# SpaceLearner/SessionRec-pytorch

Hardware: AMD Instinct MI355X
Metric: sessions/sec training, Yoochoose-1/64 batch 512 (higher is better)
Workload: dtype bf16 (MFMA operands; fp32 accumulate, master weights, scoring); 1 GPU; MSGIFSR training step, synthetic Yoochoose-1/64 shape (V=37484 items, d=256, batch 512 per GPU, session length<=20, order 3, dropout 0.1); global_batch=512, parallelism=single GPU

## Files before the change

### include/srec.h

```cpp
#ifndef SREC_H
#define SREC_H
#include "srec_hg.h"

#ifdef __cplusplus
extern "C" {
#endif

#define SREC_BAD_ARG 1001

int srec_gemm_f32(const float* A, int a_rs, int a_cs, const float* B, int b_rs, int b_cs, float* C, int ldc,
                  const float* bias, int M, int N, int K, const int* dyn, int dyn_mode, float alpha, float beta,
                  float* ws, long ws_floats, void* stream);

int srec_gemm_bf16_nt(const float* A, int lda, const float* B, int ldb, float* C, int ldc, const float* bias, int M,
                      int N, int K, const int* dyn, float alpha, float beta, float* ws, long ws_floats, void* stream);

int srec_gemm_bf16_tn(const float* A, int lda, const float* B, int ldb, float* C, int ldc, int Mred, int N, int K,
                      const int* dyn, float alpha, float beta, float* ws, long ws_floats, void* stream);

int srec_ce_plan(int B, int V, int d, int* n_item_tiles, int* n_ranges);
int srec_score_ce_fwd(const float* sr, int ld_sr, const float* E, int ld_e, const float* cs, const int* labels,
                      int B, int V, int d, const int* dynB, float* ws_stats, float* lab_logit, float* lse,
                      float* lossvec, float* loss, void* stream);
int srec_score_ce_bwd(const float* sr, int ld_sr, const float* E, int ld_e, const float* cs, const int* labels,
// ... 152 lines not shown
int srec_adam_hyper_multi(int n, const void* counter, const void* cfg, const void* hyper, const int* tap_counter,
                          const float* tap_src, float* tap_ring, int tap_n, const int* skip, void* stream);
typedef struct srec_adam_multi_desc {
    int nt;
    const int* use_wd;
    const long* numel;
    float* const* p;
    const float* const* g;
    float* const* m;
    float* const* v;
} srec_adam_multi_desc;
int srec_adam_multi(const void* desc, const float* hyper, void* stream);
int srec_adam_rows(float* W, const float* G, float* M, float* V, int n, int d, int ld, const float* hyper,
                   int use_wd, float max_norm, int renorm_write, float* cs_out, float cs_scale, int eps_mode,
                   float cs_eps, void* dst16, int Dp, void* stream);
int srec_adam_rows_proj(float* W, const float* G, float* M, float* V, int n, int d, int ld, const float* hyper, int use_wd,
                        float max_norm, int renorm_write, float* cs_out, float cs_scale, int eps_mode, float cs_eps,
                        const float* proj_cs, float proj_inv_scale, float* radial, void* dst16, int Dp, void* stream);
int srec_adam_rows_lookup(float* W, const float* G, float* M, float* V, int n, int d, int ld, const float* hyper, int use_wd,
                          float max_norm, int renorm_write, float* cs_out, float cs_scale, int eps_mode, float cs_eps,
                          const float* proj_cs, float proj_inv_scale, float* radial, void* dst16, int Dp, int* slot,
                          const float* part, const int* cptr, int u_cap, int n_part, void* stream);
int srec_adam_rows_multi(float* W, const float* G, float* M, float* V, int n, int d, int ld, const float* hyper, int use_wd,
                         float max_norm, int renorm_write, float* cs_out, float cs_scale, int eps_mode, float cs_eps,
                         const float* proj_cs, float proj_inv_scale, float* radial, void* dst16, int Dp, int* slot,
                         const float* part, const int* cptr, int u_cap, int n_part, const void* desc, const float* multi_hyper,
                         void* stream);

int srec_hg_ws_floats(const void* desc, long* n_floats);
int srec_hg_fwd(const void* desc, const float* x, int ld_x, float* out, int ld_out, unsigned char* arg, void* stream);
int srec_hg_fold(const void* desc, void* stream);
int srec_step_prep(const void* desc, void* stream);
int srec_hg_drop_prep(const float* x, const float* cnt, int rows, int D, float p, int seed, const int* counter, int salt,
                      float* ms, float* xc, float* rm, float* xres, float pa, long na, float* mk, void* stream);
int srec_hg_drop_prep16(const float* x, const float* cnt, int rows, int D, float p, int seed, const int* counter, int salt,
                        float* ms, float* xc, float* rm, float* xres, float pa, long na, float* mk, void* xc16, void* stream);
int srec_hg_live_rows(const void* desc, const void* lists, int* counts, void* stream);
int srec_hg_drop_prep16_live(const float* x, const float* cnt, int rows, int D, float p, int seed, const int* counter, int salt,
                             float* ms, float* xc, float* rm, float* xres, float pa, long na, float* mk, void* xc16,
                             const void* desc, const void* lists, int* counts, void* stream);
int srec_hg_drop_merge(const float* t, int S, const float* ms, long n, float* dx, float p, int seed, const int* counter,
                       int salt, void* stream);
int srec_hg_pre_merge(const void* desc, const float* g, int ld_g, const float* t, int S, float* dx, int ld_dx, void* stream);
int srec_hg_bwd(const void* desc, const float* x, int ld_x, const float* g, int ld_g, const unsigned char* arg, float* dx,
                int ld_dx, float* ws, void* stream);

int srec_gemm_group_bf16(const void* desc, int mode, void* stream);

int srec_gemm_f32_group_run(const void* desc, float* ws, long ws_floats, void* stream);
int srec_gemm_f32_group_run_defer(const void* desc, float* ws, long ws_floats, long* slab_off, int* slab_n, void* stream);
int srec_gemm16_nt(const void* desc, void* stream);
int srec_gemm16_nt_rows(const void* desc, const void* rows, void* stream);
int srec_gemm16_tn(const void* desc, void* stream);
int srec_rows_bf16(const float* src, int ld, int n, const int* dyn, int d, void* dst16, void* stream);
int srec_sum_slabs(const float* part, int C, int R, long n, float* out, void* stream);
int srec_weights_bf16(int n, const void* W, const void* W16, const void* WT16, const int* R, const int* Cc, void* stream);
int srec_norm_perm_pick_fwd(const float* x, int ld_x, const int* perm, int n_cap, const int* dyn_t, int D, int eps_mode,
                            float eps, float* allf, float* invr, int npick, int B, const int* dyn_b, const void* pick,
                            const void* pout, const int* ld_p, void* stream);
int srec_norm_perm_pick_bwd(const float* allf, const float* invr, const float* g_allf, int ld_g, const int* perm, int n_cap,
                            const int* cat_seg, int B, const int* dyn_b, int D, int npick, const void* pick, const void* g_pick,
                            const int* ld_gp, float* dx, int ld_dx, int nt, const int* row0, const int* ncap, const void* dyn_n,
                            int n_rows, void* stream);
int srec_gru_step_fwd(const void* desc, void* stream);
int srec_gru_step_bwd(const void* desc, void* stream);
int srec_gru_fused_fwd(const void* desc, void* stream);
int srec_gru_wfrag(int n, const void* W, const void* dst, int d, void* stream);
int srec_gru_fused_bwd(const void* desc, void* stream);
int srec_gru_fused_nodes(int np, const int* n, int d, int* nodes);
int srec_gru_fused_wide(int np, const int* n, const int* k, int* mask);
int srec_gru_fused_waves(int d, int* waves);
int srec_gru_wfrag_t(int n, const void* W, const void* dst, int d, void* stream);
int srec_gru_wfrag_both(int n, const void* W, const void* dst_fwd, const void* dst_bwd, int d, void* stream);
int srec_gru_bias_final(int np, const void* part, const int* rows, int ncol, const void* out, void* stream);
int srec_sum_slabs_multi(int np, const void* part, const int* R, const long* n, const void* out, const int* tall,
                         void* stream);
int srec_sum_slabs_multi_ld(int np, const void* part, const int* R, const long* n, const void* out, const int* tall,
                            const int* w, const int* ld, void* stream);
int srec_sum_slabs_multi_hyper(int np, const void* part, const int* R, const long* n, const void* out, const int* tall,
                               const int* w, const int* ld, int nh, const void* counter, const void* cfg, const void* hyper,
                               const int* tap_counter, const float* tap_src, float* tap_ring, int tap_n, const int* skip,
                               void* stream);

int srec_score_topk_ws(int B, int V, int K, long* bytes);
int srec_score_topk(const float* sr, int ld_sr, const float* E, int ld_e, const float* cs, int B, int V, int d, int K,
                    float* out_val, int* out_idx, void* ws, void* stream);

#define SREC_LISTED_SCORE 0
#define SREC_LISTED_DROP 1
typedef struct srec_served {
    const float* sr; int ld_sr; long comp_stride;
    const float* E; int ld_e;
    const float* cs;
    const float* off_ex; const float* off_in;
    const int* listed; int L; int listed_mode;
    long id_lo;
    int B, V, d, C;
    const float* bias; long ld_bias;
    const int* group; int G;
} srec_served;

int srec_score_rank_ws(int B, int V, int d, int C, int L, long* bytes);
int srec_score_rank(const void* served, const int* labels, float* target, int target_given, int* rank, void* ws,
                    void* stream);

#define SREC_SELECT_MAXK 128
// ... 55 lines not shown
```

### sessionrec-pytorch_amd/csrc/gemm16.hip

```cpp
#include "common.h"
#include "../../include/srec_hg.h"

namespace {

typedef __bf16 bf16x8 __attribute__((ext_vector_type(8)));
typedef short short2_t __attribute__((ext_vector_type(2)));
constexpr int G16_MAXP = 16, G16_MAXS = 4;

struct G16Args {
    const unsigned short* A[G16_MAXP][G16_MAXS];
    const unsigned short* B[G16_MAXP][G16_MAXS];
    void* C[G16_MAXP];
    const int* dyn[G16_MAXP];
    const int* rows[G16_MAXP];
    int M[G16_MAXP], N[G16_MAXP], K[G16_MAXP], nseg[G16_MAXP], koff[G16_MAXP], nsplit[G16_MAXP], start[G16_MAXP + 1];
    int np, lda, ldb, ldc;
    int ldap[G16_MAXP], ldbp[G16_MAXP], ldcp[G16_MAXP];
    float beta;
    int keep_dead;
    int per_xcd;
    int xcd_gs;
};

__device__ __forceinline__ unsigned lds_addr(const void* p) {
// ... 231 lines not shown
                for (int q4 = 0; q4 < 4; ++q4) {
                    const int idx = q4 * 64 + lane, rl = idx >> 3, c4 = (idx & 7) * 4;
                    const int row = m0 + wm * (TM / 2) + i * 32 + rl, col = n0 + wn * (TN / WN) + j * 32 + c4;
                    if (row < M && col < N) {
                        float4* q = reinterpret_cast<float4*>(C + (size_t)row * g.ldcp[p] + col);
                        if (row < Ml) {
                            float4 v = *reinterpret_cast<const float4*>(patch + rl * PS + c4);
                            if (g.beta != 0.f) {
                                const float4 o = *q;
                                v.x += g.beta * o.x; v.y += g.beta * o.y; v.z += g.beta * o.z; v.w += g.beta * o.w;
                            }
                            *q = v;
                        } else if (g.beta == 0.f) {
                            *q = make_float4(0.f, 0.f, 0.f, 0.f);
                        }
                    }
                }
                __builtin_amdgcn_wave_barrier();
            }
        return;
    }
#pragma unroll
    for (int i = 0; i < IM; ++i)
#pragma unroll
        for (int j = 0; j < IN; ++j) {
            const int col = n0 + wn * (TN / WN) + j * 32 + l31;
            if (col >= N) continue;
#pragma unroll
            for (int r = 0; r < 16; ++r) {
                const int row = m0 + wm * (TM / 2) + i * 32 + (r & 3) + 8 * (r >> 2) + 4 * half;
                if (row < M) {
                    float* q = C + (size_t)row * g.ldcp[p] + col;
                    if (row < Ml) *q = g.beta != 0.f ? acc[i][j][r] + g.beta * *q : acc[i][j][r];
                    else if (g.beta == 0.f) *q = 0.f;
                }
            }
        }
#ifdef SREC_G16_TIMING
    asm volatile("s_waitcnt vmcnt(0)" ::: "memory");
    G16T(7);
    if (threadIdx.x == 0 && bid < 8192) g_g16_blk[bid][1] = __builtin_amdgcn_s_memrealtime();
    if (threadIdx.x == 0 && bid == 17) { g_g16_tim[0] = g16t[1] - g16t[0]; g_g16_tim[1] = g16w; g_g16_tim[2] = g16d; g_g16_tim[3] = g16c; g_g16_tim[4] = g16t[7] - g16t[6]; g_g16_tim[5] = g16t[7] - g16t[0]; g_g16_tim[6] = total; }
#endif
}

typedef short short4_t __attribute__((ext_vector_type(4)));
__device__ __forceinline__ uint2 lds_tr16(const unsigned short* base, unsigned byte_off) {
    const short4_t v = __builtin_amdgcn_ds_read_tr16_b64_v4i16(
        (__attribute__((address_space(3))) short4_t*)(reinterpret_cast<const char*>(base) + byte_off));
    return __builtin_bit_cast(uint2, v);
}

template <int BR, int NS>
__global__ __launch_bounds__(256) void gemm16_tn_kernel(G16Args g) {
    constexpr int T = 128;
    constexpr int PD = NS - 1;
    constexpr int STG = 2 * BR * T;
    constexpr int NIO = BR / 4;
    constexpr int IPS = 2 * NIO / 4;
    extern __shared__ __attribute__((aligned(16))) unsigned short smem[];
    const int bid = xcd_tile(g);
    if (bid >= g.start[g.np]) return;
    int p = 0;
#pragma unroll
    for (int i = 1; i < G16_MAXP; ++i)
        if (i < g.np && bid >= g.start[i]) p = i;
    const int N1 = g.M[p], N2 = g.N[p];
    const int tn = (N2 + T - 1) / T, ntile = ((N1 + T - 1) / T) * tn;
    const int split = (bid - g.start[p]) / ntile, tile = (bid - g.start[p]) % ntile;
    const int i0 = (tile / tn) * T, j0 = (tile % tn) * T;
    const int Klive = g.dyn[p] == nullptr ? g.K[p] : max(0, min(g.K[p], *g.dyn[p] - g.koff[p]));
    const int chunk = ((Klive + g.nsplit[p] - 1) / g.nsplit[p] + 63) / 64 * 64;
    const int kbeg = split * chunk, klen = max(0, min(chunk, g.K[p] - kbeg));
    const int Kr = g.dyn[p] == nullptr ? klen : max(0, min(klen, *g.dyn[p] - g.koff[p] - kbeg));
    const int tid = threadIdx.x, lane = tid & 63;
    const int wave = __builtin_amdgcn_readfirstlane(tid >> 6);
    const int wm = wave >> 1, wn = wave & 1, half = lane >> 5, l31 = lane & 31;
    float* __restrict__ C = static_cast<float*>(g.C[p]) + (size_t)split * N1 * g.ldcp[p];

    f32x16 acc[2][2];
#pragma unroll
    for (int i = 0; i < 2; ++i)
#pragma unroll
        for (int j = 0; j < 2; ++j)
#pragma unroll
            for (int r = 0; r < 16; ++r) acc[i][j][r] = 0.f;

    const int nst = (Kr + BR - 1) / BR;
    const int total = nst * g.nseg[p];
    const unsigned lds0 = lds_addr(smem);
    const int rl = lane >> 4, sl = lane & 15;
    auto stage = [&](int it) {
        const int s = it / nst, r0 = (it - s * nst) * BR;
        const unsigned dst = lds0 + (unsigned)((it % NS) * STG) * 2u;
        const int pc = sl ^ (4 * rl);
#pragma unroll
        for (int ii = 0; ii < IPS; ++ii) {
            const int i = ii * 4 + wave;
            const int gr = kbeg + min(r0 + 4 * (i % NIO) + rl, Kr - 1);
            if (i < NIO) glds16(g.A[p][s], ((unsigned)gr * (unsigned)g.ldap[p] + (unsigned)min(i0 + pc * 8, N1 - 8)) * 2u, dst + (unsigned)i * 1024u);
            else glds16(g.B[p][s], ((unsigned)gr * (unsigned)g.ldbp[p] + (unsigned)min(j0 + pc * 8, N2 - 8)) * 2u, dst + (unsigned)i * 1024u);
        }
    };
    const int ti = lane & 15, tr = ti >> 2;
    const int tcol = 16 * ((lane >> 4) & 1) + 4 * (ti & 3);
    auto tr_off = [&](int col, int row) {
        return (unsigned)(row * 256 + ((((col >> 3) ^ (4 * (row & 3))) << 4) | ((col & 7) << 1)));
    };

    for (int s = 0; s < PD && s < total; ++s) stage(s);
    for (int it = 0; it < total; ++it) {
        wait_stage<IPS, PD>(min(total - it - 1, PD - 1));
        __syncthreads();
        if (it + PD < total) stage(it + PD);
        const int r0 = (it % nst) * BR;
// ... 32 lines not shown
            }
#pragma unroll
            for (int i = 0; i < 2; ++i)
#pragma unroll
                for (int j = 0; j < 2; ++j)
                    acc[i][j] = __builtin_amdgcn_mfma_f32_32x32x16_bf16(a[i], b[j], acc[i][j], 0, 0, 0);
        }
    }
    if ((N2 & 3) == 0 && (g.ldcp[p] & 3) == 0 && ((uintptr_t)C & 15) == 0) {
        constexpr int PS = 36;
        __syncthreads();
        float* patch = reinterpret_cast<float*>(smem) + wave * (32 * PS);
#pragma unroll
        for (int i = 0; i < 2; ++i)
#pragma unroll
            for (int j = 0; j < 2; ++j) {
#pragma unroll
                for (int r = 0; r < 16; ++r) patch[((r & 3) + 8 * (r >> 2) + 4 * half) * PS + l31] = acc[i][j][r];
                __builtin_amdgcn_wave_barrier();
                __builtin_amdgcn_s_waitcnt(0xc07f);
#pragma unroll
                for (int q4 = 0; q4 < 4; ++q4) {
                    const int idx = q4 * 64 + lane, rl = idx >> 3, c4 = (idx & 7) * 4;
                    const int row = i0 + wm * 64 + i * 32 + rl, col = j0 + wn * 64 + j * 32 + c4;
                    if (row < N1 && col < N2) {
                        float4* q = reinterpret_cast<float4*>(C + (size_t)row * g.ldcp[p] + col);
                        float4 v = *reinterpret_cast<const float4*>(patch + rl * PS + c4);
                        if (g.beta != 0.f) {
                            const float4 o = *q;
                            v.x += g.beta * o.x; v.y += g.beta * o.y; v.z += g.beta * o.z; v.w += g.beta * o.w;
                        }
                        *q = v;
                    }
                }
                __builtin_amdgcn_wave_barrier();
            }
        return;
    }
#pragma unroll
    for (int i = 0; i < 2; ++i)
#pragma unroll
        for (int j = 0; j < 2; ++j) {
            const int col = j0 + wn * 64 + j * 32 + l31;
            if (col >= N2) continue;
#pragma unroll
            for (int r = 0; r < 16; ++r) {
                const int row = i0 + wm * 64 + i * 32 + (r & 3) + 8 * (r >> 2) + 4 * half;
                if (row < N1) {
                    float* q = C + (size_t)row * g.ldcp[p] + col;
                    *q = g.beta != 0.f ? acc[i][j][r] + g.beta * *q : acc[i][j][r];
                }
            }
        }
}

__global__ void rows_bf16_kernel(const float* __restrict__ src, int ld, int n, const int* __restrict__ dyn, int d,
                                 unsigned short* __restrict__ dst) {
    const int nl = dyn_count(dyn, n);
    const long i = ((long)blockIdx.x * blockDim.x + threadIdx.x) * 4;
    if (i >= (long)n * d) return;
    const int r = (int)(i / d), c = (int)(i % d);
    float4 v = make_float4(0.f, 0.f, 0.f, 0.f);
    if (r < nl) v = *reinterpret_cast<const float4*>(src + (size_t)r * ld + c);
    uint2 o;
    o.x = srec_pack_bf16(v.x, v.y); o.y = srec_pack_bf16(v.z, v.w);
    *reinterpret_cast<uint2*>(dst + i) = o;
}

__global__ void sum_slabs_kernel(const float* __restrict__ part, int R, long n, float* __restrict__ out) {
    const long i = ((long)blockIdx.x * blockDim.x + threadIdx.x) * 4;
    if (i >= n) return;
    const float* pc = part + (size_t)blockIdx.y * R * n;
    float4 s = *reinterpret_cast<const float4*>(pc + i);
    for (int r = 1; r < R; ++r) {
        const float4 v = *reinterpret_cast<const float4*>(pc + (size_t)r * n + i);
        s.x += v.x; s.y += v.y; s.z += v.z; s.w += v.w;
    }
    *reinterpret_cast<float4*>(out + (size_t)blockIdx.y * n + i) = s;
}

int fill(G16Args& g, const void* desc_, int tm, int tn, bool tnmode, int& blocks) {
    const srec_gemm16_group* d = (const srec_gemm16_group*)desc_;
    if (d == nullptr || d->np <= 0 || d->np > G16_MAXP || (d->lda & 7) || (d->ldb & 7)) return SREC_BAD_ARG;
    g.np = d->np; g.lda = d->lda; g.ldb = d->ldb; g.ldc = d->ldc; g.beta = d->beta;
    g.keep_dead = (d->c16 & SREC_G16_KEEP_DEAD) ? 1 : 0;
    blocks = 0;
    for (int p = 0; p < d->np; ++p) {
        if (d->nseg[p] <= 0 || d->nseg[p] > G16_MAXS || d->M[p] <= 0 || d->N[p] <= 0 || d->K[p] <= 0) return SREC_BAD_ARG;
        if (!tnmode && (d->K[p] & 31)) return SREC_BAD_ARG;
        if (tnmode && ((d->M[p] & 7) || (d->N[p] & 7) || d->M[p] < 8 || d->N[p] < 8)) return SREC_BAD_ARG;
        g.M[p] = d->M[p]; g.N[p] = d->N[p]; g.K[p] = d->K[p]; g.nseg[p] = d->nseg[p]; g.C[p] = d->C[p]; g.dyn[p] = d->dyn[p];
        g.ldap[p] = d->lda_p[p] > 0 ? d->lda_p[p] : d->lda; g.ldbp[p] = d->ldb_p[p] > 0 ? d->ldb_p[p] : d->ldb;
        g.ldcp[p] = d->ldc_p[p] > 0 ? d->ldc_p[p] : d->ldc;
        if ((g.ldap[p] & 7) || (g.ldbp[p] & 7)) return SREC_BAD_ARG;
        g.koff[p] = tnmode ? d->koff[p] : 0;
        g.nsplit[p] = tnmode && d->nsplit[p] > 1 ? d->nsplit[p] : 1;
        if (g.koff[p] < 0 || g.nsplit[p] > 64) return SREC_BAD_ARG;
        for (int s = 0; s < d->nseg[p]; ++s) {
            if (((uintptr_t)d->A[p][s] & 15) || ((uintptr_t)d->B[p][s] & 15)) return SREC_BAD_ARG;
            g.A[p][s] = (const unsigned short*)d->A[p][s]; g.B[p][s] = (const unsigned short*)d->B[p][s];
        }
        g.start[p] = blocks;
        blocks += cdiv(d->M[p], tm) * cdiv(d->N[p], tn) * g.nsplit[p];
    }
    g.start[d->np] = blocks;
    return 0;
// ... 56 lines not shown
    } while (0)
#define SREC_G16(TMV, TNV, C16V, BKV, NSV, slot) SREC_G16_RL(TMV, TNV, C16V, BKV, NSV, false, slot)
    const bool deep = blocks <= 384;
    if (listed) {
        if (tn == 64) SREC_G16_RL(64, 64, true, 64, 2, true, 8);
        else if (tm == 128) SREC_G16_RL(128, 128, true, 32, 3, true, 9);
        else SREC_G16_RL(64, 128, true, 32, 3, true, 10);
    } else if (tn == 64) {
        if (c16) SREC_G16(64, 64, true, 64, 2, 0); else if (deep) SREC_G16(64, 64, false, 64, 4, 1); else SREC_G16(64, 64, false, 64, 2, 2);
    } else if (deep && tm == 64 && !c16) {
        SREC_G16(64, 128, false, 64, 4, 3);
    } else if (tm == 128) {
        if (c16) SREC_G16(128, 128, true, 32, 3, 4); else SREC_G16(128, 128, false, 64, 2, 5);
    } else {
        if (c16) SREC_G16(64, 128, true, 32, 3, 6); else SREC_G16(64, 128, false, 64, 2, 7);
    }
#undef SREC_G16
#undef SREC_G16_RL
    SREC_LAUNCH_CHECK();
    return 0;
}

extern "C" int srec_gemm16_nt(const void* desc_, void* stream) { return gemm16_nt_run(desc_, nullptr, stream); }

extern "C" int srec_gemm16_nt_rows(const void* desc_, const void* rows, void* stream) {
    return gemm16_nt_run(desc_, (const int* const*)rows, stream);
}

#ifdef SREC_G16_TIMING
extern "C" int srec_g16_timing(unsigned long long* tim8, unsigned long long* blk) {
    if (hipMemcpyFromSymbol(tim8, HIP_SYMBOL(g_g16_tim), sizeof(unsigned long long) * 8) != hipSuccess) return 1;
    return hipMemcpyFromSymbol(blk, HIP_SYMBOL(g_g16_blk), sizeof(unsigned long long) * 16384) == hipSuccess ? 0 : 1;
}
extern "C" int srec_g16_timing_reset() {
    static unsigned long long z[16384];
    return hipMemcpyToSymbol(HIP_SYMBOL(g_g16_blk), z, sizeof(z)) == hipSuccess ? 0 : 1;
}
#endif

extern "C" int srec_gemm16_tn(const void* desc_, void* stream) {
    G16Args g{};
    int blocks = 0;
    if (int rc = fill(g, desc_, 128, 128, true, blocks)) return rc;
    g.per_xcd = cdiv(blocks, 8); blocks = 8 * g.per_xcd;
    hipStream_t st = (hipStream_t)stream;
    static std::atomic<unsigned long long> om;
    const size_t lds = (size_t)2 * 2 * 64 * 128 * 2;
    if (int rc = optin(gemm16_tn_kernel<64, 2>, (int)lds, om)) return rc;
    hipLaunchKernelGGL((gemm16_tn_kernel<64, 2>), dim3(blocks), dim3(256), lds, st, g);
    SREC_LAUNCH_CHECK();
    return 0;
}

extern "C" int srec_sum_slabs(const float* part, int C, int R, long n, float* out, void* stream) {
    if (C <= 0 || R <= 0 || n <= 0) return 0;
    if (n & 3) return SREC_BAD_ARG;
    hipLaunchKernelGGL(sum_slabs_kernel, dim3((unsigned)((n / 4 + 255) / 256), C), dim3(256), 0, (hipStream_t)stream, part, R, n,
                       out);
    SREC_LAUNCH_CHECK();
    return 0;
}

extern "C" int srec_rows_bf16(const float* src, int ld, int n, const int* dyn, int d, void* dst16, void* stream) {
    if (n <= 0) return 0;
    if ((d & 3) || (ld & 3)) return SREC_BAD_ARG;
    const long items = (long)n * d / 4;
    hipLaunchKernelGGL(rows_bf16_kernel, dim3((unsigned)((items + 255) / 256)), dim3(256), 0, (hipStream_t)stream, src, ld, n,
                       dyn, d, (unsigned short*)dst16);
    SREC_LAUNCH_CHECK();
    return 0;
}
```

### sessionrec-pytorch_amd/gru.py

```python
import ctypes as _ct
from collections import namedtuple

import torch

from . import ops
from ._lib import lib, ptr, ptr_array, stream
from .ops import (G16_MAXP, GRU_MAXP, GemmProb, GruFusedBwdDesc, GruFusedDesc, GruStepDesc, _arena_rows, _arena_tag, _ld, _rows,
                  _wprep_take, can_defer, col_sum, defer_scope, defer_slab_sum, gemm16, gemm_nn, gemm_nt, gemm_tn, grad_buf,
                  grad_buf_pair, weights_bf16)


class GRUPointwise(torch.autograd.Function):

    @staticmethod
    def forward(ctx, GI, GH, bhh, Hp, dyn):
        GI = _rows(GI)
        n, d3 = GI.shape
        d = d3 // 3
        dev = GI.device
        Hn = torch.empty(n, d, device=dev, dtype=torch.float32)
        gates = torch.empty(n, d3, device=dev, dtype=torch.float32)
        if GH is not None:
            GH, Hp = _rows(GH), _rows(Hp)
            lib.srec_gru_pointwise_fwd(ptr(GI), _ld(GI), ptr(GH), _ld(GH), None, ptr(Hp), _ld(Hp), n, ptr(dyn), d,
# ... 292 lines not shown
        ctx.save_for_backward(*x16, *H, *H16, *gates, *(w for pair in wt for w in pair))
        return tuple(outs)

    @staticmethod
    def backward(ctx, *gs):
        orders, d, fused, tags, _ = ctx.meta
        P = len(orders)
        x16, H, H16, gates, wt = _saved(ctx)
        d3, dev, st = 3 * d, H[0].device, stream()
        gs = [g.contiguous() if g is not None else torch.zeros(o.n, d, device=dev) for o, g in zip(orders, gs)]
        rows = [o.n * o.k for o in orders]
        if all(t is not None for t in tags):
            dX = [_arena_rows(t, r, d, dev) for t, r in zip(tags, rows)]
        else:
            dX = pieces(torch.empty(sum(rows), d, device=dev, dtype=torch.float32), rows)
        dGI16 = [torch.empty(r, d3, device=dev, dtype=torch.bfloat16) for r in rows]
        dGH16 = [torch.empty(max(o.k - 1, 1), o.n, d3, device=dev, dtype=torch.bfloat16) for o in orders]
        if fused:
            nr, ns_c = _ct.c_int(0), (_ct.c_int * P)(*[o.n for o in orders])
            lib.srec_gru_fused_nodes(P, _ct.addressof(ns_c), d, _ct.addressof(nr))
            part = [torch.empty(-(-o.n // nr.value), 6 * d, device=dev, dtype=torch.float32) for o in orders]
            q = gru_fused_bwd_desc(orders, d, gates, H, gs, wt, dGI16, dGH16, dX, part)
            lib.srec_gru_fused_bwd(_ct.addressof(q), st)
        else:
            part = [torch.empty(o.k * gru_step_blocks(o.n, d), 6 * d, device=dev, dtype=torch.float32) for o in orders]
            dH = {}
            for t in range(max(o.k for o in orders) - 1, -1, -1):
                act = [p for p in range(P) if t < orders[p].k]
                dHp = {p: torch.empty(orders[p].n, d, device=dev, dtype=torch.float32) for p in act} if t > 0 else {}
                bufs = [StepBwd(gates[p], H[p], gs[p], dX[p], dGI16[p], dGH16[p], part[p], dH.get(p), dHp.get(p)) for p in act]
                q = gru_step_desc([(orders[p], b) for p, b in zip(act, bufs)], t, d, backward=True)
                lib.srec_gru_step_bwd(_ct.addressof(q), st)
                if t > 0:
                    gemm16('nt', [(orders[p].n, d, d3, [(dGH16[p][t - 1], wt[p][1])], dHp[p], orders[p].dyn_n) for p in act],
                           d3, d3, d, beta=1.0)
                dH = dHp
            gemm16('nt', [(rows[p], d, d3, [(dGI16[p], wt[p][0])], dX[p], o.dyn_rows) for p, o in enumerate(orders)], d3, d3, d,
                   beta=1.0)
        return GRUExpandAll._weight_grads(ctx, x16, H16, dGI16, dGH16, part, dX)

    @staticmethod
    def _weight_grads(ctx, x16, H16, dGI16, dGH16, part, dX):
        orders, d, defer = ctx.meta.orders, ctx.meta.d, ctx.meta.defer
        P = len(orders)
        d3, dev, st = 3 * d, dX[0].device, stream()
        probs, slabs = [], []
        gWih = [grad_buf(o.Wih) for o in orders]
        gWhh = [grad_buf(o.Whh) for o in orders]
        for p, o in enumerate(orders):
            hh = [(dGH16[p][t - 1], H16[p][t - 1]) for t in range(1, o.k)]
            for gW, nrow, segs, dyn in ((gWih[p], o.n * o.k, [(dGI16[p], x16[p])], o.dyn_rows), (gWhh[p], o.n, hh, o.dyn_n)):
                nsp = max(1, (nrow + 511) // 512)
                sl = torch.empty(nsp, d3, d, device=dev, dtype=torch.float32) if nsp > 1 else gW.unsqueeze(0)
                probs.append(GemmProb(d3, d, nrow, segs, sl, dyn, nsplit=nsp))
                if nsp > 1:
                    slabs.append((sl, gW))
        for i in range(0, len(probs), G16_MAXP):
            gemm16('tn', probs[i:i + G16_MAXP], d3, d, d)
        gb = [grad_buf_pair(o.bih, o.bhh) for o in orders]
        ok = can_defer(defer, [w for o in orders for w in (o.Wih, o.Whh)])
        for sl, o_ in slabs:
            defer_slab_sum(sl, o_, ok)
        if ok and can_defer(defer, [b for o in orders for b in (o.bih, o.bhh)]):
            for p in range(P):
                defer_slab_sum(part[p], gb[p], True, tall=True)
        else:
            a_p, a_o = ptr_array(part), ptr_array(gb)
            a_r = (_ct.c_int * P)(*[t_.shape[0] for t_ in part])
            lib.srec_gru_bias_final(P, _ct.addressof(a_p), _ct.addressof(a_r), 6 * d, _ct.addressof(a_o), st)
        grads = [g for p in range(P) for g in (gWih[p], gb[p][:d3], gWhh[p], gb[p][d3:])]
        return (None, None, None) + tuple(dX) + tuple(grads)


def gru_expand_all(xs, grus, ks, dyn_ns, dyn_rows):
    params = [w for g in grus for w in (g.weight_ih_l0, g.bias_ih_l0, g.weight_hh_l0, g.bias_hh_l0)]
    return GRUExpandAll.apply(tuple(ks), tuple(dyn_ns), tuple(dyn_rows), *xs, *params)
```

### sessionrec-pytorch_amd/hgat.py

```python
import ctypes as _ct
from collections import namedtuple

import torch

from . import ops
from ._lib import CONST, lib, ptr, ptr_array, stream
from .ops import GemmProb, HgDesc, _ld, _rows

DropState = namedtuple('DropState', 'xc xres mk ms rng cnt')


class HgPlan:

    def __init__(self, H, D, slope, B, dynB, types, modules, blocks, insts, mod_conv=None, layer_id=0, live=None):
        self.mod_conv = mod_conv if mod_conv is not None else [0] * len(modules)
        self.layer_id, self.live = layer_id, dict(live or {})
        self.H, self.D, self.slope, self.B, self.dynB = H, D, slope, B, dynB
        self.types, self.modules, self.blocks, self.insts, self._fold = types, modules, blocks, insts, None
        assert (len(types) <= CONST['SREC_HG_MAXT'] and len(modules) <= CONST['SREC_HG_MAXM'] and
                len(blocks) <= CONST['SREC_HG_MAXB'] and len(insts) <= CONST['SREC_HG_MAXI'])

    def put_fold(self, small, lay):
        self._fold = (small, lay)

# ... 167 lines not shown
    ws = _HG_WS.get(key)
    if ws is None:
        ws = _HG_WS[key] = torch.empty(max(n.value, 1), device=x.device, dtype=torch.float32)
    lib.srec_hg_bwd(_ct.addressof(desc), ptr(x), _ld(x), ptr(g), _ld(g), ptr(arg), ptr(dx), x.shape[1], ptr(ws), stream())
    return desc, dP, grads, dx


def _backward_data(ctx, dP, params, dx):
    plan, strategy, drop = ctx.plan, ctx.strategy, ctx.drop
    NT, D = dx.shape
    HD, nt = plan.H * D, len(plan.types)
    tgts, S, full = None, 1, False
    if drop is not None:
        nproj = {len(plan.projectors(cv, t)) for cv in (0, 1) for t in range(nt)}
        full = strategy != 'plain' and min(nproj) > 0
        if strategy == 'g16' and full and len(nproj) == 1 and 1 < min(nproj) <= 4:
            S = min(nproj)
        tgts = (torch.empty if full else torch.zeros)(2, S, NT, D, device=dx.device, dtype=torch.float32)
    beta, convs = 0.0 if full else 1.0, (0, 1) if drop is not None else (None,)
    tgt = lambda cv, j=0: dx if cv is None else tgts[cv, j]
    if strategy == 'plain':
        for cv in convs:
            for m, (r0, nr, dyn) in enumerate(plan.modules):
                if cv is None or plan.mod_conv[m] == cv:
                    ops.gemm_nn(dP[m], _rows(params[4 * m]), tgt(cv)[r0:r0 + nr], dyn, 1 if dyn is not None else 0, beta=1.0)
        return tgts, S
    W = ctx.g16[1] if strategy == 'g16' else params[::4]

    def problems(cv):
        out = []
        for t, (t0, nc, dyn_t, _) in enumerate(plan.types):
            mods = plan.projectors(cv, t)
            for j, grp in enumerate([[m] for m in mods] if S > 1 else [mods] if mods else []):
                segs = [(dP[m][t0 - plan.modules[m][0]:][:nc], W[m]) for m in grp]
                out.append(GemmProb(nc, D, HD, segs, tgt(cv, j)[t0:t0 + nc], dyn_t, mhint=plan.live.get(t0, 0)))
        return out
    if strategy == 'grouped':
        for probs in filter(None, map(problems, convs)):
            ops.gemm_group(1, probs, HD, D, D, beta=beta, a16=True)
    else:
        probs = [q for cv in convs for q in problems(cv)]
        for i in range(0, len(probs), ops.G16_MAXP):
            ops.gemm16('nt', probs[i:i + ops.G16_MAXP], HD, HD, D, beta=beta)
    return tgts, S


def _weight_grads(ctx, x, dP, gWs):
    plan, D, HD, nm = ctx.plan, x.shape[1], ctx.plan.H * x.shape[1], len(ctx.plan.modules)
    xin = [ctx.drop.xc[cv] for cv in plan.mod_conv] if ctx.drop is not None else [x] * nm
    if ctx.strategy == 'g16':
        xin16 = ctx.g16[0]
        pcs = [plan.pieces(m) for m in range(nm)]
        slabs = {m: torch.empty(len(pcs[m]), HD, D, device=x.device, dtype=torch.float32) for m in range(nm) if len(pcs[m]) > 1}
        probs = [GemmProb(HD, D, nc, [(dP[m][o:o + nc], xin16[m][t0:t0 + nc])], slabs[m][pi:pi + 1] if m in slabs else gWs[m], dyn_t)
                 for m in range(nm) for pi, (o, t0, nc, dyn_t) in enumerate(pcs[m])]
        for i in range(0, len(probs), ops.G16_MAXP):
            ops.gemm16('tn', probs[i:i + ops.G16_MAXP], HD, D, D)
        if slabs and ops.can_defer(ctx.defer, [ctx.wparams[m] for m in slabs]):
            for m, sl in slabs.items():
                ops.defer_slab_sum(sl, gWs[m])
        elif slabs:
            ops._launch_slab_sums([(sl, gWs[m]) for m, sl in slabs.items()])
    elif ctx.strategy == 'grouped':
        ops.gemm_group(2, [(HD, D, nr, [(dP[m], xin[m][r0:r0 + nr])], gWs[m], dyn)
                           for m, (r0, nr, dyn) in enumerate(plan.modules)], HD, D, D, a16=True)
    else:
        for m, (r0, nr, dyn) in enumerate(plan.modules):
            ops.gemm_tn(dP[m], xin[m][r0:r0 + nr], gWs[m], dyn)


class HGATLayer(torch.autograd.Function):

    @staticmethod
    def forward(ctx, x, plan, drop, *params):
        x = _rows(x)
        (NT, D), dev, nm = x.shape, x.device, len(plan.modules)
        strategy = gemm_strategy(ops.PRECISION['matmul'], D, _ld(x), nm, all(params[4 * m].is_contiguous() for m in range(nm)))
        dstate, x16 = None, None
        fold = plan.take_fold()
        small, lay = fold or plan.scratch(dev)
        P = [torch.empty(nr, plan.H * D, device=dev, dtype=torch.float32 if strategy == 'plain' else torch.bfloat16)
             for (r0, nr, dyn) in plan.modules]
        flat = [p.reshape(-1) if i % 4 else p for i, p in enumerate(params)]
        desc = plan.fill(HgDesc(), small, lay, P, None, flat, None, None)
        if fold is not None:
            desc.p16 |= CONST['SREC_HG_FOLDED']
        live = plan.live_rows(small, lay) if strategy == 'g16' and ops.HG_LIVE_ROWS and plan.blocks else None
        dropping = drop is not None and (drop[0] > 0 or drop[1] > 0)
        if dropping:
            x = x.contiguous()
            dstate, x16 = _drop_prep(x, plan, drop, strategy, (desc,) + live if live is not None else None)
            plan.fill_drop(desc, dstate)
        elif live is not None:
            la = ptr_array(live[0])
            lib.srec_hg_live_rows(_ct.addressof(desc), _ct.addressof(la), ptr(live[1]), stream())
        xin = [dstate.xc[cv] for cv in plan.mod_conv] if dstate is not None else [x] * nm
        g16 = _project(xin, x16, plan, params, strategy, P, live)
        out = torch.empty(NT, D, device=dev, dtype=torch.float32)
        arg = torch.empty(NT, D, device=dev, dtype=torch.uint8)
        lib.srec_hg_fwd(_ct.addressof(desc), ptr(x), _ld(x), ptr(out), D, ptr(arg), stream())
        ctx.save_for_backward(x, small, arg, *P, *params)
        ctx.plan, ctx.lay, ctx.strategy, ctx.drop, ctx.g16 = plan, lay, strategy, dstate, g16
        ctx.defer, ctx.wparams = ops.defer_scope(), [params[4 * m] for m in range(nm)]
        return out

    @staticmethod
    def backward(ctx, g):
        plan, drop, nm = ctx.plan, ctx.drop, len(ctx.plan.modules)
        x, small, arg, *rest = ctx.saved_tensors
        P, params = rest[:nm], rest[nm:]
# ... 18 lines not shown
```

### sessionrec-pytorch_amd/ops.py

```python
import ctypes as _ct
import os
from collections import namedtuple

import torch

from ._lib import CONST, STRUCTS, lib, ptr, ptr_array, stream
from .stepq import StepQueue

HgDesc = STRUCTS['srec_hg_desc']
GemmGroup = STRUCTS['srec_gemm_group']
GemmGroup16 = STRUCTS['srec_gemm16_group']
GemmF32Group = STRUCTS['srec_gemm_f32_group']
GruStepDesc = STRUCTS['srec_gru_step_desc']
GruFusedDesc = STRUCTS['srec_gru_fused_desc']
GruFusedBwdDesc = STRUCTS['srec_gru_fused_bwd_desc']
HeadDesc = STRUCTS['srec_head_desc']
HeadBwdDesc = STRUCTS['srec_head_bwd_desc']
StepPrepDesc = STRUCTS['srec_step_prep_desc']
G16_MAXP, GEMM32_MAXP, GRU_MAXP = CONST['SREC_G16_MAXP'], CONST['SREC_GEMM32_MAXP'], CONST['SREC_GRU_MAXP']
HEAD_MAXH, HEAD_MAXW = CONST['SREC_HEAD_MAXH'], CONST['SREC_HEAD_MAXW']


def _rows(t):
    assert t.dim() == 2 and t.dtype == torch.float32, (t.shape, t.dtype)
# ... 572 lines not shown
            g = _rows(g)
            ar = _arange(idx.numel() + 1, g.device)
            lib.srec_scatter_add_sorted(ptr(g), _ld(g), ptr(idx), ptr(ar), ptr(ar), ptr(gx), d, idx.numel(),
                                        ptr(ctx.dyn_b), d, 1, stream())
        return (gx, None, None, None, None) + (None,) * len(picks)


def permute_and_pick(x, perm, inv, picks, dyn_n=None, dyn_b=None):
    outs = PermuteAndPick.apply(x, perm, inv, dyn_n, dyn_b, *picks)
    for o in outs[1:]:
        o._srec_cat_left = True
    return outs[0], list(outs[1:])


def defer_scope():
    return STEP.may_defer


def can_defer(flag, params):
    if not flag:
        return False
    for q in params:
        if not q.is_leaf:
            return False
        if q.grad is not None or getattr(q, '_backward_hooks', None) or getattr(q, '_post_accumulate_grad_hooks', None):
            return False
    return True


def _launch_slab_sums(tasks, rider=None):
    for i in range(0, len(tasks), 32):
        chunk = tasks[i:i + 32]
        m = len(chunk)
        arr = _ct.c_void_p * m
        a_p, a_o = arr(*[t[0].data_ptr() for t in chunk]), arr(*[t[1].data_ptr() for t in chunk])
        a_r, a_n = (_ct.c_int * m)(*[t[0].shape[0] for t in chunk]), (_ct.c_long * m)(*[t[1].numel() for t in chunk])
        a_t = (_ct.c_int * m)(*[int(len(t) > 2 and bool(t[2])) for t in chunk])
        wl = [(0, 0) if t[1].is_contiguous() else (t[1].shape[1], t[1].stride(0)) for t in chunk]
        for t, (w, ld) in zip(chunk, wl):
            assert w == 0 or (t[1].dim() == 2 and t[1].stride(1) == 1), (t[1].shape, t[1].stride())
        a_w, a_l = (_ct.c_int * m)(*[w for w, _ in wl]), (_ct.c_int * m)(*[ld for _, ld in wl])
        if rider is not None and i + 32 >= len(tasks):
            lib.srec_sum_slabs_multi_hyper(m, _ct.addressof(a_p), _ct.addressof(a_r), _ct.addressof(a_n), _ct.addressof(a_o),
                                           _ct.addressof(a_t), _ct.addressof(a_w), _ct.addressof(a_l), *rider, stream())
        else:
            lib.srec_sum_slabs_multi_ld(m, _ct.addressof(a_p), _ct.addressof(a_r), _ct.addressof(a_n), _ct.addressof(a_o),
                                        _ct.addressof(a_t), _ct.addressof(a_w), _ct.addressof(a_l), stream())


def _launch_intake(box, M, counter, dst, cap, err):
    lib.srec_copy_words_mailbox(box, M, counter, dst, cap, err, stream())


STEP = StepQueue(_launch_slab_sums, _launch_intake)
defer_slab_sum = STEP.defer_slab_sum
flush_deferred = STEP.flush
drop_stale_deferred = STEP.drop_stale
flush_intake = STEP.flush_intake


_GRAD_EPOCH = [0]


def grad_epoch():
    _GRAD_EPOCH[0] += 1


def grad_slot(p, numel=None):
    slot = getattr(p, '_srec_gslot', None)
    if slot is None or slot[2] == _GRAD_EPOCH[0] or p.grad is not None or not p.is_leaf:
        return None
    if getattr(p, '_backward_hooks', None) or getattr(p, '_post_accumulate_grad_hooks', None):
        return None
    n = p.numel() if numel is None else numel
    if slot[1] + n > slot[0].numel():
        return None
    slot[2] = _GRAD_EPOCH[0]
    return slot[0][slot[1]:slot[1] + n]


def grad_buf(p, like=None):
    like = p if like is None else like
    v = grad_slot(p) if like.numel() == p.numel() else None
    if v is not None:
        return v.view(like.shape)
    return torch.empty(like.shape, device=like.device, dtype=torch.float32)


def grad_buf_pair(p, q):
    sp, sq = getattr(p, '_srec_gslot', None), getattr(q, '_srec_gslot', None)
    if sp is not None and sq is not None and sp[0] is sq[0] and sq[1] == sp[1] + p.numel() and sq[2] != _GRAD_EPOCH[0] \
            and q.grad is None and q.is_leaf and not getattr(q, '_backward_hooks', None) \
            and not getattr(q, '_post_accumulate_grad_hooks', None):
        v = grad_slot(p, p.numel() + q.numel())
        if v is not None:
            sq[2] = _GRAD_EPOCH[0]
            return v
    return torch.empty(p.numel() + q.numel(), device=p.device, dtype=torch.float32)


class GradMark(torch.autograd.Function):

    @staticmethod
    def forward(ctx, x, fn):
        ctx.fn = fn
        return x.view_as(x)

# ... 717 lines not shown
```

### sessionrec-pytorch_amd/stepq.py

```python
import contextlib

import torch


class StepQueue:

    def __init__(self, launch_slab_sums, launch_intake):
        self._launch_slab_sums, self._launch_intake = launch_slab_sums, launch_intake
        self._on, self._depth = False, 0
        self._sums, self._intake = [], []
        self._rider, self._done = None, None

    @property
    def may_defer(self):
        return self._on

    @contextlib.contextmanager
    def deferring(self, on):
        prev = self._on
        if not self._depth:
            self.drop_stale()
        self._depth += 1
        self._on = bool(on)
        try:
            yield
        finally:
            self._depth -= 1
            self._on = prev

    def defer_slab_sum(self, part, out, ok=True, tall=False):
        if ok and not self._sums:
            try:
                torch.autograd.Variable._execution_engine.queue_callback(self.finish)
            except RuntimeError:
                ok = False
        if not ok:
            self._launch_slab_sums([(part, out, tall)])
            return
        self._sums.append((part, out.detach(), tall))

    def waiting(self):
        return len(self._sums)

    def drop_stale(self):
        self._sums = []

    def flush(self):
        if self._sums:
            tasks, self._sums = self._sums, []
            self._launch_slab_sums(tasks, None)

    def finish(self):
        if self._sums:
            tasks, self._sums = self._sums, []
            rider, self._rider = self._rider, None
            self._launch_slab_sums(tasks, rider[0] if rider is not None else None)
            if rider is not None:
                self._done = rider[1]

    def offer_rider(self, args, slots, keepalive=None):
        self._rider, self._done = (args, frozenset(slots), keepalive), None

    def rider_result(self):
        done, self._rider, self._done = self._done, None, None
        return done

    def offer_intake(self, entries):
        self._intake = list(entries)

    def intake_pending(self):
        return bool(self._intake)

    def flush_intake(self):
        while self._intake:
            self._launch_intake(*self._intake.pop(0)[:6])

    def take_intake(self):
        box = self._intake.pop() if self._intake else None
        self.flush_intake()
        return box

    def abort(self):
        self._sums, self._intake, self._rider, self._done = [], [], None, None
```

Before: 705,000 sessions/s.

## Defer HGAT weight-grad GEMMs and launch with GRU wgrad in one kernel

The HGAT weight-gradient TN GEMMs are queued instead of launched immediately. They are later issued together with the GRU weight-gradient GEMMs through a new two-family TN kernel that interleaves tiles across the 8 XCDs. The aim is to cut kernel launch count and fill the GPU better with two small GEMM families at once. In exchange, the step queue gains more bookkeeping, weight-grad buffers are detached, and correctness depends on the queue being flushed at backward finish.

```diff
diff --git a/include/srec.h b/include/srec.h
--- a/include/srec.h
+++ b/include/srec.h
@@ -228,6 +228,7 @@
 int srec_gemm16_nt(const void* desc, void* stream);
 int srec_gemm16_nt_rows(const void* desc, const void* rows, void* stream);
 int srec_gemm16_tn(const void* desc, void* stream);
+int srec_gemm16_tn2(const void* desc_a, const void* desc_b, int b_first, void* stream);
 int srec_rows_bf16(const float* src, int ld, int n, const int* dyn, int d, void* dst16, void* stream);
 int srec_sum_slabs(const float* part, int C, int R, long n, float* out, void* stream);
 int srec_weights_bf16(int n, const void* W, const void* W16, const void* WT16, const int* R, const int* Cc, void* stream);
diff --git a/sessionrec-pytorch_amd/csrc/gemm16.hip b/sessionrec-pytorch_amd/csrc/gemm16.hip
--- a/sessionrec-pytorch_amd/csrc/gemm16.hip
+++ b/sessionrec-pytorch_amd/csrc/gemm16.hip
@@ -307,15 +307,13 @@
 }
 
 template <int BR, int NS>
-__global__ __launch_bounds__(256) void gemm16_tn_kernel(G16Args g) {
+__device__ __forceinline__ void gemm16_tn_tile(const G16Args& g, const int bid) {
     constexpr int T = 128;
     constexpr int PD = NS - 1;
     constexpr int STG = 2 * BR * T;
     constexpr int NIO = BR / 4;
     constexpr int IPS = 2 * NIO / 4;
     extern __shared__ __attribute__((aligned(16))) unsigned short smem[];
-    const int bid = xcd_tile(g);
-    if (bid >= g.start[g.np]) return;
     int p = 0;
 #pragma unroll
     for (int i = 1; i < G16_MAXP; ++i)
@@ -454,6 +452,29 @@
                 }
             }
         }
+}
+
+template <int BR, int NS>
+__global__ __launch_bounds__(256) void gemm16_tn_kernel(G16Args g) {
+    const int bid = xcd_tile(g);
+    if (bid >= g.start[g.np]) return;
+    gemm16_tn_tile<BR, NS>(g, bid);
+}
+
+struct G16Fam { int n, per, base; };
+struct G16Args2 {
+    G16Args g;
+    G16Fam first, second;
+};
+
+template <int BR, int NS>
+__global__ __launch_bounds__(256) void gemm16_tn2_kernel(G16Args2 a) {
+    const int x = (int)blockIdx.x & 7, l = (int)blockIdx.x >> 3;
+    const bool lead = l < a.first.per;
+    const G16Fam f = lead ? a.first : a.second;
+    const int t = x * f.per + (lead ? l : l - a.first.per);
+    if (t >= f.n) return;
+    gemm16_tn_tile<BR, NS>(a.g, f.base + t);
 }
 
 __global__ void rows_bf16_kernel(const float* __restrict__ src, int ld, int n, const int* __restrict__ dyn, int d,
@@ -616,6 +637,36 @@
     return 0;
 }
 
+extern "C" int srec_gemm16_tn2(const void* desc_a, const void* desc_b, int b_first, void* stream) {
+    G16Args2 a{};
+    G16Args b{};
+    G16Args& g = a.g;
+    int na = 0, nb = 0;
+    if (int rc = fill(g, desc_a, 128, 128, true, na)) return rc;
+    if (int rc = fill(b, desc_b, 128, 128, true, nb)) return rc;
+    if (g.np + b.np > G16_MAXP || g.beta != b.beta) return SREC_BAD_ARG;
+    for (int p = 0; p < b.np; ++p) {
+        const int q = g.np + p;
+        for (int s = 0; s < G16_MAXS; ++s) { g.A[q][s] = b.A[p][s]; g.B[q][s] = b.B[p][s]; }
+        g.C[q] = b.C[p]; g.dyn[q] = b.dyn[p];
+        g.M[q] = b.M[p]; g.N[q] = b.N[p]; g.K[q] = b.K[p]; g.nseg[q] = b.nseg[p]; g.koff[q] = b.koff[p]; g.nsplit[q] = b.nsplit[p];
+        g.ldap[q] = b.ldap[p]; g.ldbp[q] = b.ldbp[p]; g.ldcp[q] = b.ldcp[p];
+        g.start[q] = na + b.start[p];
+    }
+    g.np += b.np;
+    g.start[g.np] = na + nb;
+    const G16Fam fa = {na, cdiv(na, 8), 0}, fb = {nb, cdiv(nb, 8), na};
+    a.first = b_first ? fb : fa; a.second = b_first ? fa : fb;
+    const int blocks = 8 * (fa.per + fb.per);
+    hipStream_t st = (hipStream_t)stream;
+    static std::atomic<unsigned long long> om;
+    const size_t lds = (size_t)2 * 2 * 64 * 128 * 2;
+    if (int rc = optin(gemm16_tn2_kernel<64, 2>, (int)lds, om)) return rc;
+    hipLaunchKernelGGL((gemm16_tn2_kernel<64, 2>), dim3(blocks), dim3(256), lds, st, a);
+    SREC_LAUNCH_CHECK();
+    return 0;
+}
+
 extern "C" int srec_sum_slabs(const float* part, int C, int R, long n, float* out, void* stream) {
     if (C <= 0 || R <= 0 || n <= 0) return 0;
     if (n & 3) return SREC_BAD_ARG;
diff --git a/sessionrec-pytorch_amd/gru.py b/sessionrec-pytorch_amd/gru.py
--- a/sessionrec-pytorch_amd/gru.py
+++ b/sessionrec-pytorch_amd/gru.py
@@ -368,11 +368,14 @@
             for gW, nrow, segs, dyn in ((gWih[p], o.n * o.k, [(dGI16[p], x16[p])], o.dyn_rows), (gWhh[p], o.n, hh, o.dyn_n)):
                 nsp = max(1, (nrow + 511) // 512)
                 sl = torch.empty(nsp, d3, d, device=dev, dtype=torch.float32) if nsp > 1 else gW.unsqueeze(0)
-                probs.append(GemmProb(d3, d, nrow, segs, sl, dyn, nsplit=nsp))
+                probs.append(GemmProb(d3, d, nrow, segs, sl, dyn, nsplit=nsp, ld=(d3, d, d)))
                 if nsp > 1:
                     slabs.append((sl, gW))
-        for i in range(0, len(probs), G16_MAXP):
-            gemm16('tn', probs[i:i + G16_MAXP], d3, d, d)
+        if ops.WGRAD_ONE_LAUNCH and len(probs) <= G16_MAXP:
+            ops.STEP.leave_with(probs, G16_MAXP)
+        else:
+            for i in range(0, len(probs), G16_MAXP):
+                gemm16('tn', probs[i:i + G16_MAXP], d3, d, d)
         gb = [grad_buf_pair(o.bih, o.bhh) for o in orders]
         ok = can_defer(defer, [w for o in orders for w in (o.Wih, o.Whh)])
         for sl, o_ in slabs:
diff --git a/sessionrec-pytorch_amd/hgat.py b/sessionrec-pytorch_amd/hgat.py
--- a/sessionrec-pytorch_amd/hgat.py
+++ b/sessionrec-pytorch_amd/hgat.py
@@ -243,10 +243,16 @@
         xin16 = ctx.g16[0]
         pcs = [plan.pieces(m) for m in range(nm)]
         slabs = {m: torch.empty(len(pcs[m]), HD, D, device=x.device, dtype=torch.float32) for m in range(nm) if len(pcs[m]) > 1}
-        probs = [GemmProb(HD, D, nc, [(dP[m][o:o + nc], xin16[m][t0:t0 + nc])], slabs[m][pi:pi + 1] if m in slabs else gWs[m], dyn_t)
+        wait = ops.WGRAD_ONE_LAUNCH and 0 < sum(map(len, pcs)) <= ops.G16_MAXP and ops.can_defer(ctx.defer, ctx.wparams)
+        gC = [g.detach() for g in gWs] if wait else gWs
+        probs = [GemmProb(HD, D, nc, [(dP[m][o:o + nc], xin16[m][t0:t0 + nc])], slabs[m][pi:pi + 1] if m in slabs else gC[m], dyn_t,
+                          ld=(HD, D, D))
                  for m in range(nm) for pi, (o, t0, nc, dyn_t) in enumerate(pcs[m])]
-        for i in range(0, len(probs), ops.G16_MAXP):
-            ops.gemm16('tn', probs[i:i + ops.G16_MAXP], HD, D, D)
+        if wait:
+            ops.STEP.defer_product(probs, (dP, xin16, slabs))
+        else:
+            for i in range(0, len(probs), ops.G16_MAXP):
+                ops.gemm16('tn', probs[i:i + ops.G16_MAXP], HD, D, D)
         if slabs and ops.can_defer(ctx.defer, [ctx.wparams[m] for m in slabs]):
             for m, sl in slabs.items():
                 ops.defer_slab_sum(sl, gWs[m])
diff --git a/sessionrec-pytorch_amd/ops.py b/sessionrec-pytorch_amd/ops.py
--- a/sessionrec-pytorch_amd/ops.py
+++ b/sessionrec-pytorch_amd/ops.py
@@ -648,7 +648,22 @@
     lib.srec_copy_words_mailbox(box, M, counter, dst, cap, err, stream())
 
 
-STEP = StepQueue(_launch_slab_sums, _launch_intake)
+WGRAD_ONE_LAUNCH = os.environ.get('SREC_WGRAD_ONE_LAUNCH', '1') != '0'
+WGRAD_FAMILY_ORDER = os.environ.get('SREC_WGRAD_FAMILY_ORDER', 'b')
+
+
+def _launch_tn_products(fam_a, fam_b=None):
+    if fam_a and fam_b:
+        assert WGRAD_FAMILY_ORDER in ('a', 'b'), WGRAD_FAMILY_ORDER
+        ga, gb = gemm16_desc(fam_a, *fam_a[0].ld), gemm16_desc(fam_b, *fam_b[0].ld)
+        lib.srec_gemm16_tn2(_ct.addressof(ga), _ct.addressof(gb), int(WGRAD_FAMILY_ORDER == 'b'), stream())
+        return
+    probs = fam_a or fam_b
+    for i in range(0, len(probs), G16_MAXP):
+        gemm16('tn', probs[i:i + G16_MAXP], *probs[0].ld)
+
+
+STEP = StepQueue(_launch_slab_sums, _launch_intake, _launch_tn_products)
 defer_slab_sum = STEP.defer_slab_sum
 flush_deferred = STEP.flush
 drop_stale_deferred = STEP.drop_stale
diff --git a/sessionrec-pytorch_amd/stepq.py b/sessionrec-pytorch_amd/stepq.py
--- a/sessionrec-pytorch_amd/stepq.py
+++ b/sessionrec-pytorch_amd/stepq.py
@@ -5,10 +5,11 @@
 
 class StepQueue:
 
-    def __init__(self, launch_slab_sums, launch_intake):
-        self._launch_slab_sums, self._launch_intake = launch_slab_sums, launch_intake
+    def __init__(self, launch_slab_sums, launch_intake, launch_products=None):
+        self._launch_slab_sums, self._launch_intake, self._launch_products = launch_slab_sums, launch_intake, launch_products
         self._on, self._depth = False, 0
         self._sums, self._intake = [], []
+        self._products = []
         self._rider, self._done = None, None
 
     @property
@@ -28,13 +29,18 @@
             self._depth -= 1
             self._on = prev
 
+    def _in_backward(self):
+        if self._sums or self._products:
+            return True
+        try:
+            torch.autograd.Variable._execution_engine.queue_callback(self.finish)
+        except RuntimeError:
+            return False
+        return True
+
     def defer_slab_sum(self, part, out, ok=True, tall=False):
-        if ok and not self._sums:
-            try:
-                torch.autograd.Variable._execution_engine.queue_callback(self.finish)
-            except RuntimeError:
-                ok = False
-        if not ok:
+        if not (ok and self._in_backward()):
+            self._issue_products()
             self._launch_slab_sums([(part, out, tall)])
             return
         self._sums.append((part, out.detach(), tall))
@@ -43,14 +49,43 @@
         return len(self._sums)
 
     def drop_stale(self):
-        self._sums = []
+        self._sums, self._products = [], []
+
+    def defer_product(self, probs, keepalive=None, ok=True):
+        if ok and self._in_backward():
+            self._products.append((list(probs), keepalive))
+        else:
+            self._launch_products(list(probs), None)
+
+    def products_waiting(self):
+        return len(self._products)
+
+    def leave_with(self, probs, maxp):
+        waiting, self._products = self._products, []
+        room, taken, rest = maxp - len(probs), [], []
+        for e in waiting:
+            if len(e[0]) <= room:
+                taken.append(e)
+                room -= len(e[0])
+            else:
+                rest.append(e)
+        for e in rest:
+            self._launch_products(e[0], None)
+        self._launch_products([q for e in taken for q in e[0]] or None, list(probs))
+
+    def _issue_products(self):
+        waiting, self._products = self._products, []
+        for e in waiting:
+            self._launch_products(e[0], None)
 
     def flush(self):
+        self._issue_products()
         if self._sums:
             tasks, self._sums = self._sums, []
             self._launch_slab_sums(tasks, None)
 
     def finish(self):
+        self._issue_products()
         if self._sums:
             tasks, self._sums = self._sums, []
             rider, self._rider = self._rider, None
@@ -81,4 +116,4 @@
         return box
 
     def abort(self):
-        self._sums, self._intake, self._rider, self._done = [], [], None, None
+        self._sums, self._products, self._intake, self._rider, self._done = [], [], [], None, None
```

Result: faster. 717,700 sessions/s (median of 6 runs) (+1.8%).
